# amoretti86/PSVO

Hardware: AMD Instinct MI355X
Metric: particle-steps/sec (higher is better)
Workload: dtype f32

## Files before the change

### psvo_amd/csrc/common.h

```cpp
#pragma once
#include <cstddef>
#include <type_traits>
#include <hip/hip_runtime.h>
#include <stdint.h>

#include "../../include/psvo_hip.h"

#ifndef PSVO_L
#define PSVO_L 1
#endif
#if PSVO_L == 1
#define PSVO_LNS l1
#define PSVO_ENTRY(name) extern "C" int name
#define PSVO_L2_DECL(name) extern "C" __attribute__((visibility("hidden"))) decltype(name) name##_l2;
#elif PSVO_L == 2
#define PSVO_LNS l2
#define PSVO_ENTRY(name) extern "C" __attribute__((visibility("hidden"))) int name##_l2
#define PSVO_L2_DECL(name)
#else
#error "PSVO_L must be 1 or 2"
#endif

namespace psvo {

constexpr float kLog2e = 1.4426950408889634f;
constexpr float kLn2 = 0.6931471805599453f;
constexpr float kHalfLog2Pi = 0.9189385332046727f;
constexpr int kWave = 64;

extern thread_local hipError_t g_last_hip_error;
inline void clear_hip_error() { (void)hipGetLastError(); }
inline int launch_status() {
    const hipError_t e = hipGetLastError();
    if (e != hipSuccess) g_last_hip_error = e;
    return e == hipSuccess ? PSVO_OK : PSVO_ERR_HIP;
}

inline bool desc_layers_ok(const psvo_desc* d) { return !d || (d->layers >= 0 && d->layers <= 2); }

inline bool desc_emission_ok(const psvo_desc* d, int max_emission = 1) {
    return !d || (d->emission >= 0 && d->emission <= max_emission);
}

extern int g_tune_l2_split;
extern int g_tune_filter_bwd_scan;

extern int g_tune_skew_pct;

__device__ __forceinline__ void phase_skew(int cycles) {
    unsigned hw;
    asm volatile("s_getreg_b32 %0, hwreg(HW_REG_HW_ID)" : "=s"(hw));
    if (cycles > 0 && ((hw >> 16) & 1u)) {
        for (int i = 0; i < cycles; i += 64 * 32) __builtin_amdgcn_s_sleep(32);
    }
}

inline bool mlp_layers_ok(const psvo_mlp* m) { return PSVO_L == 1 || !m || (m->Wh && m->bh); }

template <int V, int... Vs, class F>
static inline int pick(int v, F&& f) {
    if (v == V) return f(std::integral_constant<int, V>{});
    if constexpr (sizeof...(Vs) > 0) return pick<Vs...>(v, f);
    else return PSVO_ERR_UNSUPPORTED;
}
template <class F> static inline int pick_dx(int Dx, F&& f) { return pick<2, 3, 4>(Dx, f); }
template <class F> static inline int pick_dy(int Dy, F&& f) { return pick<1, 2>(Dy, f); }
template <class F> static inline int pick_m(int M, F&& f) { return pick<4, 8, 16, 32>(M, f); }
inline namespace PSVO_LNS {
template <class F> static inline int pick_h(int H, F&& f) {
#if PSVO_L == 1
    return pick<16, 32, 64>(H, f);
#else
    return pick<32, 64>(H, f);
#endif
}

template <class F> static inline int dispatch_dy_h(int Dy, int H, F&& f) {
    return pick_dy(Dy, [&](auto dy) { return pick_h(H, [&](auto h) { return f(dy, h); }); });
}
template <class F> static inline int dispatch_dy_h_m(int Dy, int H, int M, F&& f) {
    return dispatch_dy_h(Dy, H, [&](auto dy, auto h) { return pick_m(M, [&](auto m) { return f(dy, h, m); }); });
}
template <class F> static inline int dispatch_shape(int Dx, int Dy, int H, F&& f) {
    return pick_dx(Dx, [&](auto dx) { return dispatch_dy_h(Dy, H, [&](auto dy, auto h) { return f(dx, dy, h); }); });
}
template <class F> static inline int dispatch_shape_m(int Dx, int Dy, int H, int M, F&& f) {
    return pick_dx(Dx, [&](auto dx) { return dispatch_dy_h_m(Dy, H, M, [&](auto dy, auto h, auto m) { return f(dx, dy, h, m); }); });
}
}

static inline int wr_cluster(int B, int N, int M) {
    int K = 8;
    while (K > 1 && ((long long)B * K > 256 || N < 4 * K || (N + K - 1) / K * (K - 1) >= N)) K >>= 1;
    (void)M;
    return K;
}

#ifdef PSVO_SECTION_TIMERS
#define PSVO_TIMERS_DEFINE(name)                                                                        \
    __device__ unsigned long long g_sec_##name[32];                                                       \
    extern "C" int psvo_debug_timers_##name(unsigned long long* out, int reset) {                         \
        if (hipMemcpyFromSymbol(out, HIP_SYMBOL(g_sec_##name), 32 * sizeof(unsigned long long)) != hipSuccess) \
            return -1;                                                                                    \
        if (reset) {                                                                                      \
            unsigned long long z[32] = {0};                                                               \
            if (hipMemcpyToSymbol(HIP_SYMBOL(g_sec_##name), z, sizeof(z)) != hipSuccess) return -1;       \
        }                                                                                                 \
        return 0;                                                                                         \
    }
#define SEC_INIT(name)                                                                          \
    unsigned long long* const _sec = g_sec_##name;                                              \
    const bool _rec = (blockIdx.x == 0 && blockIdx.y == 0 && threadIdx.x == 0);                 \
    unsigned long long _tp = clock64();
#define SEC(i)                                   \
    do {                                         \
        const unsigned long long _tn = clock64(); \
        if (_rec) _sec[i] += _tn - _tp;          \
        _tp = _tn;                               \
    } while (0)
#else
#define PSVO_TIMERS_DEFINE(name)
#define SEC_INIT(name)
#define SEC(i)
#endif

__device__ __forceinline__ float exp2_fast(float x) { return __builtin_amdgcn_exp2f(x); }
__device__ __forceinline__ float log2_fast(float x) { return __builtin_amdgcn_logf(x); }

typedef float f2 __attribute__((ext_vector_type(2)));
__device__ __forceinline__ f2 pk_fma(f2 a, f2 b, f2 c) { return __builtin_elementwise_fma(a, b, c); }
__device__ __forceinline__ f2 pk_max(f2 a, f2 b) { return __builtin_elementwise_max(a, b); }
template <int HALF>
__device__ __forceinline__ f2 pk_fma_bcast(f2 a, f2 b, f2 c) {
    f2 d;
    if constexpr (HALF == 0)
        asm("v_pk_fma_f32 %0, %1, %2, %3 op_sel_hi:[0,1,1]" : "=v"(d) : "v"(a), "v"(b), "v"(c));
    else
        asm("v_pk_fma_f32 %0, %1, %2, %3 op_sel:[1,0,0] op_sel_hi:[1,1,1]" : "=v"(d) : "v"(a), "v"(b), "v"(c));
    return d;
}

__device__ __forceinline__ void keep_in_vgpr(float& x) { asm volatile("" : "+v"(x)); }
template <int K>
__device__ __forceinline__ void keep_in_vgpr(float (&x)[K]) {
#pragma unroll
    for (int i = 0; i < K; ++i) asm volatile("" : "+v"(x[i]));
}

template <class T>
using gptr = T __attribute__((address_space(1)))*;
template <class T>
__device__ __forceinline__ gptr<T> as_global(T* p) { return (gptr<T>)p; }
template <class T>
__device__ __forceinline__ gptr<T> as_global(unsigned long long p) { return (gptr<T>)p; }
__device__ __forceinline__ float ldf(gptr<const float> base, unsigned off) {
    return *reinterpret_cast<gptr<const float>>(reinterpret_cast<gptr<const char>>(base) + off);
}
__device__ __forceinline__ int ldi(gptr<const int32_t> base, unsigned off) {
    return *reinterpret_cast<gptr<const int32_t>>(reinterpret_cast<gptr<const char>>(base) + off);
}
__device__ __forceinline__ void stf(gptr<float> base, unsigned off, float v) {
    *reinterpret_cast<gptr<float>>(reinterpret_cast<gptr<char>>(base) + off) = v;
}
__device__ __forceinline__ void sti(gptr<int32_t> base, unsigned off, int v) {
    *reinterpret_cast<gptr<int32_t>>(reinterpret_cast<gptr<char>>(base) + off) = v;
}

template <class T>
__device__ __forceinline__ T* arg_ptr(unsigned byte_off) {
    asm volatile("" : "+s"(byte_off));
    typedef const char __attribute__((address_space(4))) * kptr;
    const kptr kp = (kptr)__builtin_amdgcn_kernarg_segment_ptr();
    typedef T* const __attribute__((address_space(4))) * pptr;
    return *(pptr)(kp + byte_off);
}
template <int NPTR>
__device__ __forceinline__ void arg_block(unsigned byte_off, unsigned long long (&out)[NPTR]) {
    static_assert(NPTR == 2 || NPTR == 4 || NPTR == 8, "pointer block of 2, 4 or 8");
    asm volatile("" : "+s"(byte_off));
    typedef const char __attribute__((address_space(4))) * kptr;
    const kptr kp = (kptr)__builtin_amdgcn_kernarg_segment_ptr();
    typedef unsigned long long vec_t __attribute__((ext_vector_type(NPTR)));
    typedef const vec_t __attribute__((address_space(4))) * vptr;
    const vec_t v = *(vptr)(kp + byte_off);
#pragma unroll
    for (int i = 0; i < NPTR; ++i) out[i] = v[i];
}
#define PSVO_ARG(args_type, field) \
    ::psvo::arg_ptr<std::remove_pointer_t<decltype(args_type::field)>>((unsigned)offsetof(args_type, field))

__device__ __forceinline__ float emis_mean(float r) { return (r > 20.f ? r : log1pf(expf(r))) + 1e-6f; }
__device__ __forceinline__ float emis_dmean(float r) { return 1.f / (1.f + expf(-r)); }

template <int DIN, int H, int DOUT, int L = 1>
struct MlpLds;

template <int DIN, int H, int DOUT>
struct MlpLds<DIN, H, DOUT, 1> {
    static constexpr int kW1 = 0;
    static constexpr int kB1 = DIN * H;
    static constexpr int kW2 = kB1 + H;
    static constexpr int kB2 = kW2 + DOUT * H;
    static constexpr int kSize = kB2 + ((DOUT + 3) & ~3);

    __device__ static void load(float* __restrict__ w, const psvo_mlp& p, int tid, int nthreads) {
        for (int i = tid; i < DIN * H; i += nthreads) w[kW1 + i] = p.W1[i];
        for (int i = tid; i < H; i += nthreads) w[kB1 + i] = p.b1[i];
        for (int i = tid; i < DOUT * H; i += nthreads) {
            const int o = i / H, k = i - o * H;
            w[kW2 + i] = p.W2[k * DOUT + o];
        }
        for (int i = tid; i < ((DOUT + 3) & ~3); i += nthreads) w[kB2 + i] = i < DOUT ? p.b2[i] : 0.f;
    }

    __device__ __forceinline__ static void group4(const float* __restrict__ w, int k, const float (&x)[DIN],
                                                  f2 (&acc)[DOUT]) {
        const float4 b = *reinterpret_cast<const float4*>(w + kB1 + k);
        f2 ha = f2{b.x, b.y}, hb = f2{b.z, b.w};
#pragma unroll
        for (int i = 0; i < DIN; ++i) {
            const float4 wi = *reinterpret_cast<const float4*>(w + kW1 + i * H + k);
            const f2 xi = f2{x[i], x[i]};
            ha = pk_fma(xi, f2{wi.x, wi.y}, ha);
            hb = pk_fma(xi, f2{wi.z, wi.w}, hb);
        }
        const f2 zero = f2{0.f, 0.f};
        ha = pk_max(ha, zero);
        hb = pk_max(hb, zero);
#pragma unroll
        for (int o = 0; o < DOUT; ++o) {
            const float4 wo = *reinterpret_cast<const float4*>(w + kW2 + o * H + k);
            acc[o] = pk_fma(ha, f2{wo.x, wo.y}, acc[o]);
            acc[o] = pk_fma(hb, f2{wo.z, wo.w}, acc[o]);
        }
    }

    template <bool ROLLED = false>
    __device__ __forceinline__ static void eval(const float* __restrict__ w, const float (&x)[DIN],
                                                float (&out)[DOUT]) {
        f2 acc[DOUT];
#pragma unroll
        for (int o = 0; o < DOUT; ++o) acc[o] = f2{w[kB2 + o], 0.f};
        if constexpr (ROLLED && (H % 8 == 0) && (H > 8)) {
#pragma unroll 1
            for (int k = 0; k < H; k += 8) {
                group4(w, k, x, acc);
                group4(w, k + 4, x, acc);
            }
        } else {
#pragma unroll
            for (int k = 0; k < H; k += 4) group4(w, k, x, acc);
        }
#pragma unroll
        for (int o = 0; o < DOUT; ++o) out[o] = acc[o].x + acc[o].y;
    }

    template <int S, int PB = 0>
    __device__ __forceinline__ static void eval_part(const float* __restrict__ w, int part, const float (&x)[DIN],
                                                     float (&out)[DOUT]) {
        constexpr int HP = H / S;
        static_assert(HP % 4 == 0, "hidden slice must be a multiple of 4");
        const float* wp = w + part * HP;
        f2 acc[DOUT];
#pragma unroll
        for (int o = 0; o < DOUT; ++o) acc[o] = f2{part == 0 ? w[kB2 + o] : 0.f, 0.f};
#pragma unroll
        for (int k = 0; k < HP; k += 4) group4(wp, k, x, acc);
#pragma unroll
        for (int o = 0; o < DOUT; ++o) out[o] = acc[o].x + acc[o].y;
    }

    __device__ __forceinline__ static void bwd_group4(const float* __restrict__ w, int k, const float (&x)[DIN],
                                                      const float (&dout)[DOUT], f2 (&dxa)[DIN]) {
        const float4 b = *reinterpret_cast<const float4*>(w + kB1 + k);
        f2 pa = f2{b.x, b.y}, pb = f2{b.z, b.w};
        f2 wa[DIN], wb[DIN];
#pragma unroll
        for (int i = 0; i < DIN; ++i) {
            const float4 wi = *reinterpret_cast<const float4*>(w + kW1 + i * H + k);
            wa[i] = f2{wi.x, wi.y};
            wb[i] = f2{wi.z, wi.w};
            const f2 xi = f2{x[i], x[i]};
            pa = pk_fma(xi, wa[i], pa);
            pb = pk_fma(xi, wb[i], pb);
        }
        f2 da = f2{0.f, 0.f}, db = da;
#pragma unroll
        for (int o = 0; o < DOUT; ++o) {
            const float4 wo = *reinterpret_cast<const float4*>(w + kW2 + o * H + k);
            const f2 go = f2{dout[o], dout[o]};
            da = pk_fma(go, f2{wo.x, wo.y}, da);
            db = pk_fma(go, f2{wo.z, wo.w}, db);
        }
        da = f2{pa.x > 0.f ? da.x : 0.f, pa.y > 0.f ? da.y : 0.f};
        db = f2{pb.x > 0.f ? db.x : 0.f, pb.y > 0.f ? db.y : 0.f};
#pragma unroll
        for (int i = 0; i < DIN; ++i) {
            dxa[i] = pk_fma(da, wa[i], dxa[i]);
            dxa[i] = pk_fma(db, wb[i], dxa[i]);
        }
    }

    template <int S, int PB = 0>
    __device__ __forceinline__ static void bwd_input_part(const float* __restrict__ w, int part, const float (&x)[DIN],
                                                          const float (&dout)[DOUT], float (&dx)[DIN]) {
        constexpr int HP = H / S;
        const float* wp = w + part * HP;
        f2 dxa[DIN];
#pragma unroll
        for (int i = 0; i < DIN; ++i) dxa[i] = f2{dx[i], 0.f};
#pragma unroll
        for (int k = 0; k < HP; k += 4) bwd_group4(wp, k, x, dout, dxa);
#pragma unroll
        for (int i = 0; i < DIN; ++i) dx[i] = dxa[i].x + dxa[i].y;
    }

    template <bool ROLLED = false>
    __device__ __forceinline__ static void bwd_input(const float* __restrict__ w, const float (&x)[DIN],
                                                     const float (&dout)[DOUT], float (&dx)[DIN]) {
        f2 dxa[DIN];
#pragma unroll
        for (int i = 0; i < DIN; ++i) dxa[i] = f2{dx[i], 0.f};
        if constexpr (ROLLED && (H % 8 == 0) && (H > 8)) {
#pragma unroll 1
            for (int k = 0; k < H; k += 8) {
                bwd_group4(w, k, x, dout, dxa);
                bwd_group4(w, k + 4, x, dout, dxa);
            }
        } else {
#pragma unroll
            for (int k = 0; k < H; k += 4) bwd_group4(w, k, x, dout, dxa);
        }
#pragma unroll
        for (int i = 0; i < DIN; ++i) dx[i] = dxa[i].x + dxa[i].y;
    }
};

typedef float f4v __attribute__((ext_vector_type(4)));
template <int MASK>
__device__ __forceinline__ float xor_lane(float v);
constexpr int ilog2(int v) { return v <= 1 ? 0 : 1 + ilog2(v >> 1); }

__device__ __forceinline__ float lane_fetch(float v, int src_lane) {
    return __builtin_bit_cast(float, __builtin_amdgcn_ds_bpermute(src_lane << 2, __builtin_bit_cast(int, v)));
}

#ifdef PSVO_L2_VALU
#include "mlp2_valu.h"
#else
template <int DIN, int H, int DOUT>
struct MlpLds<DIN, H, DOUT, 2> {
    static constexpr int kW1 = 0;
    static constexpr int kB1 = DIN * H;
    static constexpr int kW2 = kB1 + H;
    static constexpr int kB2 = kW2 + DOUT * H;
    static constexpr int kWS = H + 4;
    static constexpr int kWh = kB2 + ((DOUT + 3) & ~3);
    static constexpr int kBh = kWh + H * kWS;
    static constexpr int kSize = kBh + H;
    static constexpr int NQ = H / 16;
    static_assert(H % 16 == 0, "hidden width must be a multiple of 16 (MFMA tile)");

    __device__ static void load(float* __restrict__ w, const psvo_mlp& p, int tid, int nthreads) {
        MlpLds<DIN, H, DOUT, 1>::load(w, p, tid, nthreads);
        for (int i = tid; i < H * H; i += nthreads) {
            const int k = i / H, j = i - k * H;
            w[kWh + j * kWS + k] = p.Wh[i];
        }
        for (int i = tid; i < H * (kWS - H); i += nthreads) w[kWh + (i / (kWS - H)) * kWS + H + i % (kWS - H)] = 0.f;
        for (int i = tid; i < H; i += nthreads) w[kBh + i] = p.bh[i];
    }

    template <int S, int PB>
    struct Rows {
        static constexpr int LS = (S == 1) ? 0 : (S == 2) ? 1 : (S == 4) ? 2 : (S == 8) ? 3 : (S == 16) ? 4 : (S == 32) ? 5 : 6;
        static_assert((1 << LS) == S, "lanes per row: a power of two");
        static constexpr int NR = 64 / S;
        static constexpr int NG = (NR + 15) / 16;
        static constexpr int LOW = (1 << PB) - 1;
        __device__ __forceinline__ static int row(int lane) { return ((lane >> (PB + LS)) << PB) | (lane & LOW); }
        __device__ __forceinline__ static int owner(int rho) { return ((rho >> PB) << (PB + LS)) | (rho & LOW); }
        __device__ __forceinline__ static bool owns(int lane) { return ((lane >> PB) & (S - 1)) == 0; }
    };

    __device__ __forceinline__ static void layer1(const float* __restrict__ w, int g, const float (&xr)[DIN],
                                                  float (&pre)[NQ][4]) {
#pragma unroll
        for (int q = 0; q < NQ; ++q) {
            const float4 b = *reinterpret_cast<const float4*>(w + kB1 + 16 * q + 4 * g);
            pre[q][0] = b.x; pre[q][1] = b.y; pre[q][2] = b.z; pre[q][3] = b.w;
#pragma unroll
            for (int d = 0; d < DIN; ++d) {
                const float4 wi = *reinterpret_cast<const float4*>(w + kW1 + d * H + 16 * q + 4 * g);
                pre[q][0] = fmaf(xr[d], wi.x, pre[q][0]);
                pre[q][1] = fmaf(xr[d], wi.y, pre[q][1]);
                pre[q][2] = fmaf(xr[d], wi.z, pre[q][2]);
                pre[q][3] = fmaf(xr[d], wi.w, pre[q][3]);
            }
        }
    }

    __device__ __forceinline__ static void hidden2(const float* __restrict__ w, int g, int r, const float (&pre1)[NQ][4],
                                                   f4v (&D)[NQ]) {
#pragma unroll
        for (int jt = 0; jt < NQ; ++jt) {
            const float4 b = *reinterpret_cast<const float4*>(w + kBh + 16 * jt + 4 * g);
            D[jt] = f4v{b.x, b.y, b.z, b.w};
        }
        const float* wa = w + kWh + r * kWS + 4 * g;
#pragma unroll
        for (int q = 0; q < NQ; ++q) {
            float h[4];
#pragma unroll
            for (int c = 0; c < 4; ++c) h[c] = fmaxf(pre1[q][c], 0.f);
#pragma unroll
            for (int jt = 0; jt < NQ; ++jt) {
                const float4 a4 = *reinterpret_cast<const float4*>(wa + 16 * jt * kWS + 16 * q);
                D[jt] = __builtin_amdgcn_mfma_f32_16x16x4f32(a4.x, h[0], D[jt], 0, 0, 0);
                D[jt] = __builtin_amdgcn_mfma_f32_16x16x4f32(a4.y, h[1], D[jt], 0, 0, 0);
                D[jt] = __builtin_amdgcn_mfma_f32_16x16x4f32(a4.z, h[2], D[jt], 0, 0, 0);
                D[jt] = __builtin_amdgcn_mfma_f32_16x16x4f32(a4.w, h[3], D[jt], 0, 0, 0);
            }
        }
    }

    template <int S, int PB>
    __device__ __forceinline__ static void eval_rows(const float* __restrict__ w, bool with_bias, const float (&x)[DIN],
                                                     float (&out)[DOUT]) {
        using R = Rows<S, PB>;
        const int lane = __lane_id(), g = lane >> 4, r = lane & 15;
        const int my_row = R::row(lane);
        const bool mine = R::owns(lane);
#pragma unroll
        for (int o = 0; o < DOUT; ++o) out[o] = 0.f;
#pragma unroll 1
        for (int p = 0; p < R::NG; ++p) {
            const int src = R::owner((16 * p + r) & (R::NR - 1));
            float xr[DIN];
#pragma unroll
            for (int d = 0; d < DIN; ++d) xr[d] = lane_fetch(x[d], src);
            float pre1[NQ][4];
            layer1(w, g, xr, pre1);
            f4v D[NQ];
            hidden2(w, g, r, pre1, D);
            float acc[DOUT];
#pragma unroll
            for (int o = 0; o < DOUT; ++o) acc[o] = 0.f;
#pragma unroll
            for (int jt = 0; jt < NQ; ++jt) {
                const float h0 = fmaxf(D[jt][0], 0.f), h1 = fmaxf(D[jt][1], 0.f), h2 = fmaxf(D[jt][2], 0.f),
                            h3 = fmaxf(D[jt][3], 0.f);
#pragma unroll
                for (int o = 0; o < DOUT; ++o) {
                    const float4 wo = *reinterpret_cast<const float4*>(w + kW2 + o * H + 16 * jt + 4 * g);
                    acc[o] = fmaf(h0, wo.x, fmaf(h1, wo.y, fmaf(h2, wo.z, fmaf(h3, wo.w, acc[o]))));
                }
            }
#pragma unroll
            for (int o = 0; o < DOUT; ++o) {
                float v = acc[o];
                v += xor_lane<16>(v);
                v += xor_lane<32>(v);
                const float t = lane_fetch(v, my_row & 15);
                if (mine && (my_row >> 4) == p) out[o] = t + (with_bias ? w[kB2 + o] : 0.f);
            }
        }
    }

    template <int S, int PB>
    __device__ __forceinline__ static void bwd_rows(const float* __restrict__ w, const float (&x)[DIN],
                                                    const float (&dout)[DOUT], float (&dx)[DIN]) {
        using R = Rows<S, PB>;
        const int lane = __lane_id(), g = lane >> 4, r = lane & 15;
        const int my_row = R::row(lane);
        const bool mine = R::owns(lane);
#pragma unroll 1
        for (int p = 0; p < R::NG; ++p) {
            const int src = R::owner((16 * p + r) & (R::NR - 1));
            float xr[DIN], gr[DOUT];
#pragma unroll
            for (int d = 0; d < DIN; ++d) xr[d] = lane_fetch(x[d], src);
#pragma unroll
            for (int o = 0; o < DOUT; ++o) gr[o] = lane_fetch(dout[o], src);
            float pre1[NQ][4];
            layer1(w, g, xr, pre1);
            f4v D[NQ];
            hidden2(w, g, r, pre1, D);
            float dp[NQ][4];
#pragma unroll
            for (int jt = 0; jt < NQ; ++jt) {
                float s[4] = {0.f, 0.f, 0.f, 0.f};
#pragma unroll
                for (int o = 0; o < DOUT; ++o) {
                    const float4 wo = *reinterpret_cast<const float4*>(w + kW2 + o * H + 16 * jt + 4 * g);
                    s[0] = fmaf(gr[o], wo.x, s[0]); s[1] = fmaf(gr[o], wo.y, s[1]);
                    s[2] = fmaf(gr[o], wo.z, s[2]); s[3] = fmaf(gr[o], wo.w, s[3]);
                }
#pragma unroll
                for (int v = 0; v < 4; ++v) dp[jt][v] = D[jt][v] > 0.f ? s[v] : 0.f;
            }
            f4v E[NQ];
#pragma unroll
            for (int kt = 0; kt < NQ; ++kt) E[kt] = f4v{0.f, 0.f, 0.f, 0.f};
            const float* wb = w + kWh + 4 * g * kWS + r;
#pragma unroll
            for (int jt = 0; jt < NQ; ++jt) {
#pragma unroll
                for (int v = 0; v < 4; ++v) {
#pragma unroll
                    for (int kt = 0; kt < NQ; ++kt) {
                        const float a = wb[(16 * jt + v) * kWS + 16 * kt];
                        E[kt] = __builtin_amdgcn_mfma_f32_16x16x4f32(a, dp[jt][v], E[kt], 0, 0, 0);
                    }
                }
            }
            float acc[DIN];
#pragma unroll
            for (int d = 0; d < DIN; ++d) acc[d] = 0.f;
#pragma unroll
            for (int q = 0; q < NQ; ++q) {
                float e[4];
#pragma unroll
                for (int c = 0; c < 4; ++c) e[c] = pre1[q][c] > 0.f ? E[q][c] : 0.f;
#pragma unroll
                for (int d = 0; d < DIN; ++d) {
                    const float4 wi = *reinterpret_cast<const float4*>(w + kW1 + d * H + 16 * q + 4 * g);
                    acc[d] = fmaf(e[0], wi.x, fmaf(e[1], wi.y, fmaf(e[2], wi.z, fmaf(e[3], wi.w, acc[d]))));
                }
            }
#pragma unroll
            for (int d = 0; d < DIN; ++d) {
                float v = acc[d];
                v += xor_lane<16>(v);
                v += xor_lane<32>(v);
                const float t = lane_fetch(v, my_row & 15);
                if (mine && (my_row >> 4) == p) dx[d] += t;
            }
        }
    }

    template <bool ROLLED = false>
    __device__ __forceinline__ static void eval(const float* __restrict__ w, const float (&x)[DIN], float (&out)[DOUT]) {
        eval_rows<1, 0>(w, true, x, out);
    }
    template <int S, int PB = 0>
    __device__ __forceinline__ static void eval_part(const float* __restrict__ w, int , const float (&x)[DIN],
                                                     float (&out)[DOUT]) {
        eval_rows<S, PB>(w, true, x, out);
    }
    template <bool ROLLED = false>
    __device__ __forceinline__ static void bwd_input(const float* __restrict__ w, const float (&x)[DIN],
                                                     const float (&dout)[DOUT], float (&dx)[DIN]) {
        bwd_rows<1, 0>(w, x, dout, dx);
    }
    template <int S, int PB = 0>
    __device__ __forceinline__ static void bwd_input_part(const float* __restrict__ w, int , const float (&x)[DIN],
                                                          const float (&dout)[DOUT], float (&dx)[DIN]) {
        bwd_rows<S, PB>(w, x, dout, dx);
    }
};
#endif

template <int D>
__device__ __forceinline__ float diag_lp(const float (&x)[D], const float (&mu)[D], const float (&inv_s)[D],
                                         float cst) {
    float acc = 0.f;
#pragma unroll
    for (int d = 0; d < D; ++d) {
        const float z = (x[d] - mu[d]) * inv_s[d];
        acc = fmaf(z, z, acc);
    }
    return fmaf(-0.5f, acc, cst);
}

template <int CTRL, int ROW_MASK = 0xF, int BANK_MASK = 0xF, bool BOUND = false>
__device__ __forceinline__ float dpp_mov(float old, float v) {
    return __builtin_bit_cast(float, __builtin_amdgcn_update_dpp(__builtin_bit_cast(int, old), __builtin_bit_cast(int, v),
                                                                  CTRL, ROW_MASK, BANK_MASK, BOUND));
}

template <int MASK>
__device__ __forceinline__ float xor_lane(float v) {
    static_assert(MASK == 1 || MASK == 2 || MASK == 4 || MASK == 8 || MASK == 16 || MASK == 32, "xor_lane mask");
    if constexpr (MASK == 1) {
        return dpp_mov<0xB1, 0xF, 0xF, true>(v, v);
    } else if constexpr (MASK == 2) {
        return dpp_mov<0x4E, 0xF, 0xF, true>(v, v);
    } else if constexpr (MASK == 4) {
        float t = dpp_mov<0x104, 0xF, 0x5>(v, v);
        return dpp_mov<0x114, 0xF, 0xA>(t, v);
    } else if constexpr (MASK == 8) {
        return dpp_mov<0x128, 0xF, 0xF, true>(v, v);
    } else if constexpr (MASK == 16) {
        const unsigned u = __builtin_bit_cast(unsigned, v);
        const auto p = __builtin_amdgcn_permlane16_swap(u, u, false, false);
        const bool odd_row = (__lane_id() >> 4) & 1;
        return __builtin_bit_cast(float, odd_row ? p[0] : p[1]);
    } else {
        const unsigned u = __builtin_bit_cast(unsigned, v);
        const auto p = __builtin_amdgcn_permlane32_swap(u, u, false, false);
        return __builtin_bit_cast(float, (__lane_id() >= 32) ? p[0] : p[1]);
    }
}

__device__ __forceinline__ float wave_incl_scan(float v, int ) {
    v += dpp_mov<0x111, 0xF, 0xF, true>(0.f, v);
    v += dpp_mov<0x112, 0xF, 0xF, true>(0.f, v);
    v += dpp_mov<0x114, 0xF, 0xF, true>(0.f, v);
    v += dpp_mov<0x118, 0xF, 0xF, true>(0.f, v);
    v += dpp_mov<0x142, 0xA, 0xF, false>(0.f, v);
    v += dpp_mov<0x143, 0xC, 0xF, false>(0.f, v);
    return v;
}
__device__ __forceinline__ float wave_sum(float v) {
    v = wave_incl_scan(v, 0);
    return __builtin_bit_cast(float, __builtin_amdgcn_readlane(__builtin_bit_cast(int, v), 63));
}
__device__ __forceinline__ float wave_max(float v) {
    const float ninf = -__builtin_huge_valf();
    v = fmaxf(v, dpp_mov<0x111>(ninf, v));
    v = fmaxf(v, dpp_mov<0x112>(ninf, v));
    v = fmaxf(v, dpp_mov<0x114>(ninf, v));
    v = fmaxf(v, dpp_mov<0x118>(ninf, v));
    v = fmaxf(v, dpp_mov<0x142, 0xA>(ninf, v));
    v = fmaxf(v, dpp_mov<0x143, 0xC>(ninf, v));
    return __builtin_bit_cast(float, __builtin_amdgcn_readlane(__builtin_bit_cast(int, v), 63));
}
__device__ __forceinline__ void quad_bcast4(float v, float (&out)[4]) {
    out[0] = dpp_mov<0x00>(v, v);
    out[1] = dpp_mov<0x55>(v, v);
    out[2] = dpp_mov<0xAA>(v, v);
    out[3] = dpp_mov<0xFF>(v, v);
}

typedef float __attribute__((__may_alias__)) in_word_t;

template <int NS>
__device__ __forceinline__ float quad_field(const float (&slot)[NS], int f) {
    const float v = slot[f >> 2];
    switch (f & 3) {
        case 0: return dpp_mov<0x00>(v, v);
        case 1: return dpp_mov<0x55>(v, v);
        case 2: return dpp_mov<0xAA>(v, v);
        default: return dpp_mov<0xFF>(v, v);
    }
}

template <int G>
__device__ __forceinline__ float group_sum(float v) {
    if constexpr (G > 1) v += xor_lane<1>(v);
    if constexpr (G > 2) v += xor_lane<2>(v);
    if constexpr (G > 4) v += xor_lane<4>(v);
    if constexpr (G > 8) v += xor_lane<8>(v);
    if constexpr (G > 16) v += xor_lane<16>(v);
    if constexpr (G > 32) v += xor_lane<32>(v);
    return v;
}
template <int G>
__device__ __forceinline__ float group_max(float v) {
    if constexpr (G > 1) v = fmaxf(v, xor_lane<1>(v));
    if constexpr (G > 2) v = fmaxf(v, xor_lane<2>(v));
    if constexpr (G > 4) v = fmaxf(v, xor_lane<4>(v));
    if constexpr (G > 8) v = fmaxf(v, xor_lane<8>(v));
    if constexpr (G > 16) v = fmaxf(v, xor_lane<16>(v));
    if constexpr (G > 32) v = fmaxf(v, xor_lane<32>(v));
    return v;
}
template <int G>
__device__ __forceinline__ float group_incl_scan(float v, int m) {
    if constexpr (G > 1) { const float t = dpp_mov<0x111, 0xF, 0xF, true>(0.f, v); v += (m >= 1) ? t : 0.f; }
    if constexpr (G > 2) { const float t = dpp_mov<0x112, 0xF, 0xF, true>(0.f, v); v += (m >= 2) ? t : 0.f; }
    if constexpr (G > 4) { const float t = dpp_mov<0x114, 0xF, 0xF, true>(0.f, v); v += (m >= 4) ? t : 0.f; }
    if constexpr (G > 8) { const float t = dpp_mov<0x118, 0xF, 0xF, true>(0.f, v); v += (m >= 8) ? t : 0.f; }
    if constexpr (G > 16) v += dpp_mov<0x142, 0xA, 0xF, false>(0.f, v);
    if constexpr (G > 32) v += dpp_mov<0x143, 0xC, 0xF, false>(0.f, v);
    return v;
}

__device__ __forceinline__ float lane_bcast(float v, int src) {
    return __builtin_bit_cast(float, __builtin_amdgcn_readlane(__builtin_bit_cast(int, v), src));
}

__device__ __forceinline__ float block_max(float v, float* red, int slot, int wave, int lane, int nw) {
    v = wave_max(v);
    if (nw == 1) return v;
    float* r = red + slot * 16;
    if (lane == 0) r[wave] = v;
    __syncthreads();
    float m = r[0];
    for (int i = 1; i < nw; ++i) m = fmaxf(m, r[i]);
    return m;
}
__device__ __forceinline__ float block_sum(float v, float* red, int wave, int lane, int nw) {
    v = wave_sum(v);
    if (nw == 1) return v;
    if (lane == 0) red[wave] = v;
    __syncthreads();
    float s = 0.f;
    for (int i = 0; i < nw; ++i) s += red[i];
    __syncthreads();
    return s;
}

template <int DX>
struct StepK {
    float c[DX];
    float ic[DX];
    float i1[DX];
    float i2[DX];
    float ifs[DX];
    float lq, lf;
};

template <int DX>
__device__ __forceinline__ StepK<DX> make_stepk(const float* s1, const float* s2, const float* fs, bool two_q) {
    StepK<DX> K;
    float lq = -DX * kHalfLog2Pi, lf = -DX * kHalfLog2Pi;
#pragma unroll
    for (int d = 0; d < DX; ++d) {
        K.i1[d] = 1.f / s1[d];
        if (two_q) {
            K.i2[d] = 1.f / s2[d];
            K.ic[d] = K.i1[d] + K.i2[d];
            K.c[d] = 1.f / K.ic[d];
        } else {
            K.i2[d] = 0.f;
            K.ic[d] = K.i1[d];
            K.c[d] = s1[d];
        }
        K.ifs[d] = 1.f / fs[d];
        lq -= logf(K.c[d]);
        lf -= logf(fs[d]);
    }
    K.lq = lq;
    K.lf = lf;
    return K;
}

template <int DX>
struct StepKR {
    float c[DX], ic[DX], i1[DX], i2[DX], ifs[DX];
};
template <int DX>
__device__ __forceinline__ StepKR<DX> make_stepkr(const float* s1, const float* s2, const float* fs, bool two_q) {
    StepKR<DX> K;
#pragma unroll
    for (int d = 0; d < DX; ++d) {
        K.i1[d] = 1.f / s1[d];
        if (two_q) {
            K.i2[d] = 1.f / s2[d];
            K.ic[d] = K.i1[d] + K.i2[d];
            K.c[d] = 1.f / K.ic[d];
        } else {
            K.i2[d] = 0.f;
            K.ic[d] = K.i1[d];
            K.c[d] = s1[d];
        }
        K.ifs[d] = 1.f / fs[d];
    }
    return K;
}

template <int DX>
struct FAcc {
    static constexpr int kSc = 0;
    static constexpr int kSmm1 = DX;
    static constexpr int kSmb = 2 * DX;
    static constexpr int kSmm = 3 * DX;
    static constexpr int kSfs = 4 * DX;
    static constexpr int kSet = 5 * DX;
    static constexpr int kSg = 2 * kSet;
};

template <int DX>
struct BAcc {
    static constexpr int kSc = 0;
    static constexpr int kSmm1 = DX;
    static constexpr int kSmb = 2 * DX;
    static constexpr int kSmm = 3 * DX;
    static constexpr int kSf = 4 * DX;
    static constexpr int kSinit = 5 * DX;
    static constexpr int kSiota = 6 * DX;
    static constexpr int kSg = 7 * DX;
};

__device__ __forceinline__ void pog_scale_grad(float s1, float s2, float Sc, float Smm1, float Smb, float Smm, float& ds1,
                                               float& ds2) {
    const float i1 = 1.f / s1, i2 = 1.f / s2;
    const float c = 1.f / (i1 + i2);
    const float dc = Sc + Smm / c;
    const float di1 = c * Smm1 - c * c * dc;
    const float di2 = c * Smb - c * c * dc;
    ds1 = -i1 * i1 * di1;
    ds2 = -i2 * i2 * di2;
}

void launch_row_sum(const float* in, long long rows, int L, float* out, hipStream_t stream);
void launch_reduce_rows(const float* part, int nrows, long long stride, int n, float* out, int accumulate, hipStream_t stream);
void launch_step_fold(const float* part, int T, int B, int nacc, float* sacc, hipStream_t stream);
struct FilterFinalizeArgs {
    const float* sacc;
    int B, Dy, two_q, bootstrap;
    const float *sig_q1, *sig_q2, *sig0;
    int same0;
    float *dsig_q1, *dsig_q2, *dsig_f, *dsig_g, *dsig0, *dfsig0;
};
int launch_filter_bwd_finalize(int Dx, const FilterFinalizeArgs& a, hipStream_t stream);
struct BsimFoldArgs {
    const float *dFm_part, *dlogW_part;
    int T, B, nblk, N, Dy;
    float *dFm, *dlogW, *dlse;
    const float* sacc;
    int rows;
    const float *sig_q1inv, *sig_bq2;
    float *dsig_f, *dsig_g, *dsig_q1inv, *dsig_bq2, *dsig_init, *disig;
};
int launch_bsim_bwd_fold_finalize(int Dx, const BsimFoldArgs& a, hipStream_t stream);

}
```

### psvo_amd/csrc/filter_fwd_impl.h

```cpp
#if PSVO_AD
#define PSVO_FWD_KERNEL filter_fwd_ad_kernel
#define PSVO_FWD_LPP_KERNEL filter_fwd_lpp_ad_kernel
#define PSVO_FWD_ARGS FilterArgsAd
#else
#define PSVO_FWD_KERNEL filter_fwd_kernel
#define PSVO_FWD_LPP_KERNEL filter_fwd_lpp_kernel
#define PSVO_FWD_ARGS FilterArgs
#endif

template <int DX, int DY, int H, int MAXT, int EM = 2>
__global__ void __launch_bounds__(MAXT) PSVO_FWD_KERNEL(const PSVO_FWD_ARGS a) {
    using MQ = MlpLds<DX, H, DX, PSVO_L>;
    using MG = MlpLds<DX, H, DY, PSVO_L>;
    extern __shared__ __attribute__((aligned(16))) float smem[];

    const int tid = threadIdx.x, lane = tid & 63, wave = tid >> 6;
    const int NT = blockDim.x, nw = NT >> 6;
    const int b = blockIdx.x, B = a.B, T = a.T, N = a.N;
    const bool valid = tid < N;
    const int n = valid ? tid : N - 1;

    float* wq1 = smem;
    float* wf = wq1 + MQ::kSize;
    float* wg = wf + MQ::kSize;
    float* cdf = wg + MG::kSize;
    float* sx = cdf + NT;
    float* sp = sx + DX * NT;
    float* sf = sp + DX * NT;
    float* red = sf + DX * NT;

    MQ::load(wq1, a.q1, tid, NT);
    if (!a.bootstrap) MQ::load(wf, a.f, tid, NT);
    MG::load(wg, a.g, tid, NT);
    const float* wfm = a.bootstrap ? wq1 : wf;

    float sq1[DX], sq2[DX], sfv[DX], s0[DX], fs0[DX], isg[DY];
    float lg = -DY * kHalfLog2Pi;
#pragma unroll
    for (int d = 0; d < DX; ++d) {
        sq1[d] = a.sig_q1[d];
        sq2[d] = a.two_q ? a.sig_q2[d] : 1.f;
        sfv[d] = a.bootstrap ? a.sig_q1[d] : a.sig_f[d];
        s0[d] = a.sig0[d];
        fs0[d] = a.fsig0[d];
    }
#pragma unroll
    for (int e = 0; e < DY; ++e) {
        const float s = a.sig_g[e];
        isg[e] = 1.f / s;
        lg -= logf(s);
    }
    const StepK<DX> K0 = make_stepk<DX>(s0, sq2, fs0, a.two_q != 0);
    const StepK<DX> K1 = make_stepk<DX>(sq1, sq2, sfv, a.two_q != 0);
    const float neg_logN = -logf((float)N);
    const float ninf = -__builtin_huge_valf();

    float mean1[DX], fmean[DX];
#pragma unroll
    for (int d = 0; d < DX; ++d) {
        mean1[d] = a.m0[b * DX + d];
        fmean[d] = a.fm0[b * DX + d];
    }
    float lnw = neg_logN;

    float eps_c[DX], mu2_c[DX], obs_c[DY], u_c = 0.f;
    int idx_c = 0;
    auto load_inputs = [&](int t, float (&e)[DX], float (&m)[DX], float (&o)[DY], float& uu, int& ii) {
        const size_t tb = (size_t)t * B + b;
#pragma unroll
        for (int d = 0; d < DX; ++d) {
            e[d] = a.eps[(tb * DX + d) * N + n];
            m[d] = a.two_q ? a.mu2[tb * DX + d] : 0.f;
        }
#pragma unroll
        for (int k = 0; k < DY; ++k) o[k] = a.obs[tb * DY + k];
        if (a.resample) {
            if (a.idx_in) ii = a.idx_in[tb * N + n];
            else uu = a.u[tb * N + n];
        }
    };
    load_inputs(0, eps_c, mu2_c, obs_c, u_c, idx_c);
    __syncthreads();

    constexpr int kWeights = MQ::kSize + MG::kSize;
    constexpr bool kOpaque = (MAXT > 256) ? (kWeights > 120) : (kWeights > 330);

    SEC_INIT(filter_fwd)
    for (int t = 0; t < T; ++t) {
        SEC(0);
        const size_t tb = (size_t)t * B + b;
        const StepK<DX> K = (t == 0) ? K0 : K1;
#if PSVO_AD
        int rs_f = 0;
        if (a.rs_in) rs_f = a.rs_in[tb];
#endif
        int zo = 0;
        if (kOpaque) asm volatile("" : "+v"(zo));
        const float* wq1_t = wq1 + zo;
        const float* wfm_t = wfm + zo;
        const float* wg_t = wg + zo;

        float eps_n[DX], mu2_n[DX], obs_n[DY], u_n = 0.f;
        int idx_n = 0;
        if (t + 1 < T) load_inputs(t + 1, eps_n, mu2_n, obs_n, u_n, idx_n);

        SEC(1);
        float mu[DX], x[DX];
#pragma unroll
        for (int d = 0; d < DX; ++d) {
            mu[d] = a.two_q ? K.c[d] * fmaf(K.i1[d], mean1[d], K.i2[d] * mu2_c[d]) : mean1[d];
            x[d] = fmaf(K.c[d], eps_c[d], mu[d]);
        }
        const float q_lp = diag_lp<DX>(x, mu, K.ic, K.lq);
        const float f_lp = diag_lp<DX>(x, fmean, K.ifs, K.lf);

        SEC(2);
        float gm[DY];
        MG::template eval<kOpaque>(wg_t, x, gm);
        if (EM == 2 ? (a.emission != 0) : (EM == 1)) {
#pragma unroll
            for (int k = 0; k < DY; ++k) gm[k] = emis_mean(gm[k]);
        }
        const float g_lp = diag_lp<DY>(obs_c, gm, isg, lg);

        float lw = f_lp + g_lp - q_lp + lnw;
        if (!valid) lw = ninf;

        SEC(3);
        float p1[DX], fm[DX];
        MQ::template eval<kOpaque>(wq1_t, x, p1);
        if (a.bootstrap) {
#pragma unroll
            for (int d = 0; d < DX; ++d) fm[d] = p1[d];
        } else {
            MQ::template eval<kOpaque>(wfm_t, x, fm);
        }
        if (valid) {
#pragma unroll
            for (int d = 0; d < DX; ++d) {
                a.X[(tb * DX + d) * N + n] = x[d];
                a.Fm[(tb * DX + d) * N + n] = fm[d];
                if (a.P1) a.P1[(tb * DX + d) * N + n] = p1[d];
            }
            a.logW[tb * N + n] = lw;
        }

        SEC(4);
        const float mx = block_max(lw, red, 0, wave, lane, nw);
        const float w = valid ? exp2_fast((lw - mx) * kLog2e) : 0.f;
        float sc = wave_incl_scan(w, lane);
        float total;
#if PSVO_AD
        float tot2 = wave_sum(w * w);
#endif
        if (nw > 1) {
            float* wt = red + 32;
            if (lane == 63) wt[wave] = sc;
#if PSVO_AD
            if (lane == 63) red[16 + wave] = tot2;
#endif
            __syncthreads();
            float off = 0.f, tot = 0.f;
            for (int i = 0; i < nw; ++i) {
                const float v = wt[i];
                if (i < wave) off += v;
                tot += v;
            }
            sc += off;
            total = tot;
#if PSVO_AD
            tot2 = 0.f;
            for (int i = 0; i < nw; ++i) tot2 += red[16 + i];
#endif
        } else {
            total = lane_bcast(sc, 63);
        }
        const float lse_t = fmaf(kLn2, log2_fast(total), mx);
        if (tid == 0) a.lse[tb] = lse_t;
#if PSVO_AD
        const float ess = total * total / tot2;
        const bool inherit = a.rs_in ? (rs_f != 0) : !(ess >= a.ess_frac * (float)N);
        if (tid == 0) {
            a.ess_out[tb] = ess;
            a.rs_out[tb] = inherit ? 1 : 0;
        }
#endif

        SEC(5);
        if (a.resample) {
            cdf[tid] = sc;
#pragma unroll
            for (int d = 0; d < DX; ++d) {
                sx[d * NT + tid] = x[d];
                sp[d * NT + tid] = p1[d];
                if (!a.bootstrap) sf[d * NT + tid] = fm[d];
            }
            __syncthreads();
            SEC(6);
            int idx;
            if (a.idx_in) {
                idx = idx_c;
            } else {
                const float target = u_c * total;
                int pos = 0;
                for (int s = 1 << (31 - __clz(N)); s > 0; s >>= 1) {
                    const int p = pos + s;
                    if (p <= N && cdf[p - 1] <= target) pos = p;
                }
                idx = min(pos, N - 1);
            }
#pragma unroll
            for (int d = 0; d < DX; ++d) {
                x[d] = sx[d * NT + idx];
                mean1[d] = sp[d * NT + idx];
                fmean[d] = a.bootstrap ? mean1[d] : sf[d * NT + idx];
            }
            if (valid) {
                a.idx_out[tb * N + n] = idx;
#pragma unroll
                for (int d = 0; d < DX; ++d) a.Xanc[(tb * DX + d) * N + n] = x[d];
            }
            lnw = neg_logN;
#if PSVO_AD
#pragma unroll
            for (int d = 0; d < DX; ++d) {
                mean1[d] = inherit ? mean1[d] : p1[d];
                fmean[d] = inherit ? fmean[d] : fm[d];
            }
            lnw = inherit ? neg_logN : lw - lse_t;
#endif
            SEC(7);
            __syncthreads();
        } else {
#pragma unroll
            for (int d = 0; d < DX; ++d) {
                mean1[d] = p1[d];
                fmean[d] = fm[d];
            }
            if (valid) {
                a.idx_out[tb * N + n] = n;
#pragma unroll
                for (int d = 0; d < DX; ++d) a.Xanc[(tb * DX + d) * N + n] = x[d];
            }
            lnw = lw - lse_t;
            if (nw > 1) __syncthreads();
        }

#pragma unroll
        for (int d = 0; d < DX; ++d) {
            eps_c[d] = eps_n[d];
            mu2_c[d] = mu2_n[d];
        }
#pragma unroll
        for (int k = 0; k < DY; ++k) obs_c[k] = obs_n[k];
        u_c = u_n;
        idx_c = idx_n;
    }
}

template <int DX, int DY, int H, int MAXT>
__global__ void __launch_bounds__(MAXT) PSVO_FWD_LPP_KERNEL(const PSVO_FWD_ARGS a) {
    using MQ = MlpLds<DX, H, DX, PSVO_L>;
    using MG = MlpLds<DX, H, DY, PSVO_L>;
    constexpr int P = 4;
    constexpr bool kOpaque = false;
    extern __shared__ __attribute__((aligned(16))) float smem[];

    const int tid = threadIdx.x, lane = tid & 63, wave = tid >> 6;
    const int NT = blockDim.x, nw = NT >> 6;
    const int NPT = NT / P;
    const int b = blockIdx.x, B = a.B, T = a.T, N = a.N;
    const int pn = tid >> 2, p = tid & 3;
    const int uwave = __builtin_amdgcn_readfirstlane(wave);
    const bool valid = pn < N;
    const int n = valid ? pn : N - 1;

    float* wq1 = smem;
    float* wf = wq1 + MQ::kSize;
    float* wg = wf + MQ::kSize;
    float* cdf = wg + MG::kSize;
    float* piv = cdf + NPT;
    float* sx = piv + 16;
    float* sp = sx + DX * NPT;
    float* sf = sp + DX * NPT;
    float* red = sf + DX * NPT;

    MQ::load(wq1, a.q1, tid, NT);
    if (!a.bootstrap) MQ::load(wf, a.f, tid, NT);
    MG::load(wg, a.g, tid, NT);
    const float* wfm = a.bootstrap ? wq1 : wf;
    if (tid < 16) piv[tid] = __builtin_huge_valf();

    float sq1[DX], sq2[DX], sfv[DX], s0[DX], fs0[DX], isg[DY];
    float lg = -DY * kHalfLog2Pi;
#pragma unroll
    for (int d = 0; d < DX; ++d) {
        sq1[d] = a.sig_q1[d];
        sq2[d] = a.two_q ? a.sig_q2[d] : 1.f;
        sfv[d] = a.bootstrap ? a.sig_q1[d] : a.sig_f[d];
        s0[d] = a.sig0[d];
        fs0[d] = a.fsig0[d];
    }
#pragma unroll
    for (int e = 0; e < DY; ++e) {
        const float s = a.sig_g[e];
        isg[e] = 1.f / s;
        lg -= logf(s);
    }
    const StepK<DX> K0 = make_stepk<DX>(s0, sq2, fs0, a.two_q != 0);
    const StepK<DX> K1 = make_stepk<DX>(sq1, sq2, sfv, a.two_q != 0);
    const float neg_logN = -logf((float)N);
    const float ninf = -__builtin_huge_valf();

    float mean1[DX], fmean[DX];
#pragma unroll
    for (int d = 0; d < DX; ++d) {
        mean1[d] = a.m0[b * DX + d];
        fmean[d] = a.fm0[b * DX + d];
    }
    float lnw = neg_logN;

    constexpr int kFU = DX, kFM2 = DX + 1, kFY = 2 * DX + 1, kFields = 2 * DX + 1 + DY, kSlots = (kFields + 3) / 4;
    const in_word_t* in_ptr[kSlots];
    int in_str[kSlots];
    auto field_ptr = [&](int f, const in_word_t*& q, int& st) {
        q = a.eps + (size_t)b * DX * N + n;
        st = 0;
        if (f < kFU) {
            q = a.eps + ((size_t)b * DX + f) * N + n;
            st = B * DX * N;
        } else if (f == kFU) {
            if (a.resample) {
                q = (a.idx_in ? reinterpret_cast<const in_word_t*>(a.idx_in) : static_cast<const in_word_t*>(a.u)) + (size_t)b * N + n;
                st = B * N;
            }
        } else if (f < kFY) {
            if (a.two_q) {
                q = a.mu2 + (size_t)b * DX + (f - kFM2);
                st = B * DX;
            }
        } else if (f < kFields) {
            q = a.obs + (size_t)b * DY + (f - kFY);
            st = B * DY;
        }
    };
#pragma unroll
    for (int s = 0; s < kSlots; ++s) {
        field_ptr(4 * s, in_ptr[s], in_str[s]);
#pragma unroll
        for (int j = 1; j < 4; ++j) {
            const in_word_t* q;
            int st;
            field_ptr(4 * s + j, q, st);
            in_ptr[s] = (p == j) ? q : in_ptr[s];
            in_str[s] = (p == j) ? st : in_str[s];
        }
    }
    float eps_c[DX], mu2_c[DX], obs_c[DY], u_c = 0.f;
    int idx_c = 0;
    float raw_n[kSlots];
    auto issue_inputs = [&]() {
#pragma unroll
        for (int s = 0; s < kSlots; ++s) {
            raw_n[s] = *in_ptr[s];
            in_ptr[s] += in_str[s];
        }
    };
    auto take_inputs = [&]() {
#pragma unroll
        for (int d = 0; d < DX; ++d) {
            eps_c[d] = quad_field(raw_n, d);
            const float m = quad_field(raw_n, kFM2 + d);
            mu2_c[d] = a.two_q ? m : 0.f;
        }
#pragma unroll
        for (int k = 0; k < DY; ++k) obs_c[k] = quad_field(raw_n, kFY + k);
        u_c = quad_field(raw_n, kFU);
        idx_c = __builtin_bit_cast(int, u_c);
    };
    issue_inputs();
    take_inputs();
    __syncthreads();

    SEC_INIT(filter_fwd)
    auto step = [&](auto first_tag, const int t) {
        SEC(0);
        const size_t tb = (size_t)t * B + b;
        const StepK<DX> K = decltype(first_tag)::value ? K0 : K1;
#if PSVO_AD
        int rs_f = 0;
        if (a.rs_in) rs_f = a.rs_in[tb];
#endif
        if (t + 1 < T) issue_inputs();

        SEC(1);
        float mu[DX], x[DX];
#pragma unroll
        for (int d = 0; d < DX; ++d) {
            mu[d] = a.two_q ? K.c[d] * fmaf(K.i1[d], mean1[d], K.i2[d] * mu2_c[d]) : mean1[d];
            x[d] = fmaf(K.c[d], eps_c[d], mu[d]);
        }
        const float q_lp = diag_lp<DX>(x, mu, K.ic, K.lq);
        const float f_lp = diag_lp<DX>(x, fmean, K.ifs, K.lf);

        SEC(2);
        int zo = 0;
        if (kOpaque) asm volatile("" : "+v"(zo));
        float gm[DY], p1[DX], fm[DX];
        MG::template eval_part<P>(wg + zo, p, x, gm);
        MQ::template eval_part<P>(wq1 + zo, p, x, p1);
        if (!a.bootstrap) MQ::template eval_part<P>(wfm + zo, p, x, fm);
#pragma unroll
        for (int k = 0; k < DY; ++k) gm[k] = group_sum<P>(gm[k]);
        if (a.emission) {
#pragma unroll
            for (int k = 0; k < DY; ++k) gm[k] = emis_mean(gm[k]);
        }
#pragma unroll
        for (int d = 0; d < DX; ++d) {
            p1[d] = group_sum<P>(p1[d]);
            fm[d] = a.bootstrap ? p1[d] : group_sum<P>(fm[d]);
        }
        const float g_lp = diag_lp<DY>(obs_c, gm, isg, lg);
        float lw = f_lp + g_lp - q_lp + lnw;
        if (!valid) lw = ninf;

        if (valid) {
            if (p == 0) {
#pragma unroll
                for (int d = 0; d < DX; ++d) a.X[(tb * DX + d) * N + n] = x[d];
                a.logW[tb * N + n] = lw;
            } else if (p == 1) {
#pragma unroll
                for (int d = 0; d < DX; ++d) a.Fm[(tb * DX + d) * N + n] = fm[d];
            } else if (p == 2 && a.P1) {
#pragma unroll
                for (int d = 0; d < DX; ++d) a.P1[(tb * DX + d) * N + n] = p1[d];
            }
        }

        SEC(3);
        const float wmx = wave_max(lw);
        const float wbase = (wmx == ninf) ? 0.f : wmx;
        const float w = (valid && p == 0) ? exp2_fast((lw - wbase) * kLog2e) : 0.f;
        float sc = wave_incl_scan(w, lane);
#if PSVO_AD
        const float wsq = wave_sum(w * w);
#endif
        if (lane == 63) {
            red[wave] = wmx;
            red[16 + wave] = sc;
#if PSVO_AD
            red[32 + wave] = wsq;
#endif
        }
        if (a.resample) {
            if (p == 1) {
#pragma unroll
                for (int d = 0; d < DX; ++d) sx[d * NPT + pn] = x[d];
            } else if (p == 2) {
#pragma unroll
                for (int d = 0; d < DX; ++d) sp[d * NPT + pn] = p1[d];
            } else if (p == 3 && !a.bootstrap) {
#pragma unroll
                for (int d = 0; d < DX; ++d) sf[d * NPT + pn] = fm[d];
            }
        }
        SEC(4);
        __syncthreads();
        SEC(5);
        const int li = lane & 15;
        const float m_i = li < nw ? red[li] : ninf;
        const float s_i = li < nw ? red[16 + li] : 0.f;
        const float gmx = lane_bcast(group_max<16>(m_i), 0);
        const float gbase = (gmx == ninf) ? 0.f : gmx;
        const float v_i = s_i * exp2_fast((m_i - gbase) * kLog2e);
        const float pre = group_incl_scan<16>(v_i, li);
        const float total = lane_bcast(pre, nw - 1);
        const float off = uwave > 0 ? lane_bcast(pre, max(uwave - 1, 0)) : 0.f;
        sc = fmaf(sc, exp2_fast((wbase - gbase) * kLog2e), off);
        const float lse_t = fmaf(kLn2, log2_fast(total), gmx);
        if (tid == 3) a.lse[tb] = lse_t;
#if PSVO_AD
        const float q_i = li < nw ? red[32 + li] : 0.f;
        const float r_i = exp2_fast((m_i - gbase) * kLog2e);
        const float tot2 = lane_bcast(group_incl_scan<16>(q_i * r_i * r_i, li), nw - 1);
        const float ess = total * total / tot2;
        const bool inherit = a.rs_in ? (rs_f != 0) : !(ess >= a.ess_frac * (float)N);
        if (tid == 7) {
            a.ess_out[tb] = ess;
            a.rs_out[tb] = inherit ? 1 : 0;
        }
#endif

        SEC(6);
        if (a.resample) {
            if (p == 0) {
                cdf[pn] = sc;
                if ((pn & 15) == 15) piv[pn >> 4] = sc;
            }
            __syncthreads();
            SEC(7);
            int idx;
            if (a.idx_in) {
                idx = idx_c;
            } else {
                const float target = u_c * total;
                const float4 pv = *reinterpret_cast<const float4*>(piv + 4 * p);
                float c1 = (pv.x <= target ? 1.f : 0.f) + (pv.y <= target ? 1.f : 0.f) +
                           (pv.z <= target ? 1.f : 0.f) + (pv.w <= target ? 1.f : 0.f);
                c1 = group_sum<P>(c1);
                const int blk = min((int)c1, (NPT >> 4) - 1);
                const float4 cv = *reinterpret_cast<const float4*>(cdf + 16 * blk + 4 * p);
                float c2 = (cv.x <= target ? 1.f : 0.f) + (cv.y <= target ? 1.f : 0.f) +
                           (cv.z <= target ? 1.f : 0.f) + (cv.w <= target ? 1.f : 0.f);
                c2 = group_sum<P>(c2);
                idx = min(16 * blk + (int)c2, N - 1);
            }
#pragma unroll
            for (int d = 0; d < DX; ++d) {
                x[d] = sx[d * NPT + idx];
                mean1[d] = sp[d * NPT + idx];
                fmean[d] = a.bootstrap ? mean1[d] : sf[d * NPT + idx];
            }
            if (valid) {
                if (p == 3) a.idx_out[tb * N + n] = idx;
                if (p == 0) {
#pragma unroll
                    for (int d = 0; d < DX; ++d) a.Xanc[(tb * DX + d) * N + n] = x[d];
                }
            }
            lnw = neg_logN;
#if PSVO_AD
#pragma unroll
            for (int d = 0; d < DX; ++d) {
                mean1[d] = inherit ? mean1[d] : p1[d];
                fmean[d] = inherit ? fmean[d] : fm[d];
            }
            lnw = inherit ? neg_logN : lw - lse_t;
#endif
            SEC(8);
            __syncthreads();
            SEC(9);
        } else {
#pragma unroll
            for (int d = 0; d < DX; ++d) {
                mean1[d] = p1[d];
                fmean[d] = fm[d];
            }
            if (valid) {
                if (p == 3) a.idx_out[tb * N + n] = n;
                if (p == 0) {
#pragma unroll
                    for (int d = 0; d < DX; ++d) a.Xanc[(tb * DX + d) * N + n] = x[d];
                }
            }
            lnw = lw - lse_t;
            __syncthreads();
        }

        take_inputs();
    };
    step(std::true_type{}, 0);
    for (int t = 1; t < T; ++t) step(std::false_type{}, t);
}

#undef PSVO_FWD_KERNEL
#undef PSVO_FWD_LPP_KERNEL
#undef PSVO_FWD_ARGS
```

Measured before the change: 260.9 million.

## Cache per-lane MLP weight slices in registers for the LPP forward kernel

Measured after the change: 264.0 million (median of 6 runs). +1.2%, better.

```diff
diff --git a/psvo_amd/csrc/common.h b/psvo_amd/csrc/common.h
--- a/psvo_amd/csrc/common.h
+++ b/psvo_amd/csrc/common.h
@@ -266,6 +266,66 @@
         for (int o = 0; o < DOUT; ++o) acc[o] = f2{part == 0 ? w[kB2 + o] : 0.f, 0.f};
 #pragma unroll
         for (int k = 0; k < HP; k += 4) group4(wp, k, x, acc);
+#pragma unroll
+        for (int o = 0; o < DOUT; ++o) out[o] = acc[o].x + acc[o].y;
+    }
+
+    template <int S>
+    struct Slice {
+        static constexpr int HP = H / S;
+        static constexpr int kFloats = HP * (1 + DIN + DOUT) + DOUT;
+        f2 b1[HP / 2], w1[DIN][HP / 2], w2[DOUT][HP / 2];
+        f2 acc0[DOUT];
+    };
+    template <int S>
+    __device__ __forceinline__ static void load_slice(const float* __restrict__ w, int part, Slice<S>& s) {
+        constexpr int HP = H / S;
+        static_assert(HP % 4 == 0, "hidden slice must be a multiple of 4");
+        const float* wp = w + part * HP;
+#pragma unroll
+        for (int k = 0; k < HP; k += 4) {
+            const float4 b = *reinterpret_cast<const float4*>(wp + kB1 + k);
+            s.b1[k / 2] = f2{b.x, b.y};
+            s.b1[k / 2 + 1] = f2{b.z, b.w};
+#pragma unroll
+            for (int i = 0; i < DIN; ++i) {
+                const float4 wi = *reinterpret_cast<const float4*>(wp + kW1 + i * H + k);
+                s.w1[i][k / 2] = f2{wi.x, wi.y};
+                s.w1[i][k / 2 + 1] = f2{wi.z, wi.w};
+            }
+#pragma unroll
+            for (int o = 0; o < DOUT; ++o) {
+                const float4 wo = *reinterpret_cast<const float4*>(wp + kW2 + o * H + k);
+                s.w2[o][k / 2] = f2{wo.x, wo.y};
+                s.w2[o][k / 2 + 1] = f2{wo.z, wo.w};
+            }
+        }
+#pragma unroll
+        for (int o = 0; o < DOUT; ++o) s.acc0[o] = f2{part == 0 ? w[kB2 + o] : 0.f, 0.f};
+    }
+    template <int S>
+    __device__ __forceinline__ static void eval_part(const Slice<S>& s, const float (&x)[DIN], float (&out)[DOUT]) {
+        f2 acc[DOUT];
+#pragma unroll
+        for (int o = 0; o < DOUT; ++o) acc[o] = s.acc0[o];
+        const f2 zero = f2{0.f, 0.f};
+#pragma unroll
+        for (int k = 0; k < H / S / 2; k += 2) {
+            f2 ha = s.b1[k], hb = s.b1[k + 1];
+#pragma unroll
+            for (int i = 0; i < DIN; ++i) {
+                const f2 xi = f2{x[i], x[i]};
+                ha = pk_fma(xi, s.w1[i][k], ha);
+                hb = pk_fma(xi, s.w1[i][k + 1], hb);
+            }
+            ha = pk_max(ha, zero);
+            hb = pk_max(hb, zero);
+#pragma unroll
+            for (int o = 0; o < DOUT; ++o) {
+                acc[o] = pk_fma(ha, s.w2[o][k], acc[o]);
+                acc[o] = pk_fma(hb, s.w2[o][k + 1], acc[o]);
+            }
+        }
 #pragma unroll
         for (int o = 0; o < DOUT; ++o) out[o] = acc[o].x + acc[o].y;
     }
diff --git a/psvo_amd/csrc/filter_fwd_impl.h b/psvo_amd/csrc/filter_fwd_impl.h
--- a/psvo_amd/csrc/filter_fwd_impl.h
+++ b/psvo_amd/csrc/filter_fwd_impl.h
@@ -263,7 +263,11 @@
     using MQ = MlpLds<DX, H, DX, PSVO_L>;
     using MG = MlpLds<DX, H, DY, PSVO_L>;
     constexpr int P = 4;
-    constexpr bool kOpaque = false;
+    using SG = typename MlpLds<DX, H, DY, 1>::template Slice<P>;
+    using SQ = typename MlpLds<DX, H, DX, 1>::template Slice<P>;
+    constexpr int kSliceBudget = 120;
+    constexpr bool kRegGQ = PSVO_L == 1 && DX <= 3 && !(PSVO_AD && DY == 2);
+    constexpr bool kRegF = kRegGQ && SG::kFloats + 2 * SQ::kFloats <= kSliceBudget;
     extern __shared__ __attribute__((aligned(16))) float smem[];
 
     const int tid = threadIdx.x, lane = tid & 63, wave = tid >> 6;
@@ -382,6 +386,14 @@
     take_inputs();
     __syncthreads();
 
+    SG rg;
+    SQ rq, rf;
+    if constexpr (kRegGQ) {
+        MlpLds<DX, H, DY, 1>::template load_slice<P>(wg, p, rg);
+        MlpLds<DX, H, DX, 1>::template load_slice<P>(wq1, p, rq);
+    }
+    if constexpr (kRegF) MlpLds<DX, H, DX, 1>::template load_slice<P>(wfm, p, rf);
+
     SEC_INIT(filter_fwd)
     auto step = [&](auto first_tag, const int t) {
         SEC(0);
@@ -404,12 +416,18 @@
         const float f_lp = diag_lp<DX>(x, fmean, K.ifs, K.lf);
 
         SEC(2);
-        int zo = 0;
-        if (kOpaque) asm volatile("" : "+v"(zo));
         float gm[DY], p1[DX], fm[DX];
-        MG::template eval_part<P>(wg + zo, p, x, gm);
-        MQ::template eval_part<P>(wq1 + zo, p, x, p1);
-        if (!a.bootstrap) MQ::template eval_part<P>(wfm + zo, p, x, fm);
+        if constexpr (kRegGQ) {
+            MlpLds<DX, H, DY, 1>::template eval_part<P>(rg, x, gm);
+            MlpLds<DX, H, DX, 1>::template eval_part<P>(rq, x, p1);
+        } else {
+            MG::template eval_part<P>(wg, p, x, gm);
+            MQ::template eval_part<P>(wq1, p, x, p1);
+        }
+        if (!a.bootstrap) {
+            if constexpr (kRegF) MlpLds<DX, H, DX, 1>::template eval_part<P>(rf, x, fm);
+            else MQ::template eval_part<P>(wfm, p, x, fm);
+        }
 #pragma unroll
         for (int k = 0; k < DY; ++k) gm[k] = group_sum<P>(gm[k]);
         if (a.emission) {
```
